# helgeanl/GP-MPC

Measured on NVIDIA H100. Metric: GP predictions/sec (N train x horizon test, fp64), higher is better.
Workload: dtype f64

## Files before the change

gp-mpc_b200/csrc/gpmpc.cu:

```cuda
#include "../../include/gpmpc.h"

#include <dlfcn.h>
#include <math.h>
#include <stdarg.h>
#include <stdlib.h>
#include <string.h>

#include <algorithm>
#include <type_traits>
#include <vector>

#include <nvtx3/nvToolsExt.h>

#include "common.cuh"
#include "gemm_dmma.cuh"
#include "predict_streamk.cuh"
#include "kernels.cuh"

#define GPMPC_VERSION 100
#define HB 64
#define NX_MAX 32
#define PSK_MAX_CTAS 2048
#define MAX_DEPTH 12
#define LOOKAHEAD_MIN_ROWS 1024

typedef struct { char internal[128]; } nccl_uid_t;
typedef void* nccl_comm_t;
struct NcclApi {
    void* lib = nullptr;
    int (*GetUniqueId)(nccl_uid_t*) = nullptr;
    int (*CommInitRank)(nccl_comm_t*, int, nccl_uid_t, int) = nullptr;
    int (*AllGather)(const void*, void*, size_t, int, nccl_comm_t, cudaStream_t) = nullptr;
    int (*CommDestroy)(nccl_comm_t) = nullptr;
    const char* (*GetErrorString)(int) = nullptr;
};
static NcclApi g_nccl;
static char g_create_err[512] = "";

static bool nccl_load(char* err, size_t errn)
{
    if (g_nccl.lib) return true;
    const char* names[] = {"libnccl.so.2", "libnccl.so"};
    for (const char* n : names) {
        g_nccl.lib = dlopen(n, RTLD_NOW | RTLD_GLOBAL);
        if (g_nccl.lib) break;
    }
    if (!g_nccl.lib) { snprintf(err, errn, "dlopen(libnccl.so.2) failed: %s", dlerror()); return false; }
    g_nccl.GetUniqueId = (int (*)(nccl_uid_t*))dlsym(g_nccl.lib, "ncclGetUniqueId");
    g_nccl.CommInitRank = (int (*)(nccl_comm_t*, int, nccl_uid_t, int))dlsym(g_nccl.lib, "ncclCommInitRank");
    g_nccl.AllGather = (int (*)(const void*, void*, size_t, int, nccl_comm_t, cudaStream_t))dlsym(g_nccl.lib, "ncclAllGather");
    g_nccl.CommDestroy = (int (*)(nccl_comm_t))dlsym(g_nccl.lib, "ncclCommDestroy");
    g_nccl.GetErrorString = (const char* (*)(int))dlsym(g_nccl.lib, "ncclGetErrorString");
    if (!g_nccl.GetUniqueId || !g_nccl.CommInitRank || !g_nccl.AllGather || !g_nccl.CommDestroy) {
        snprintf(err, errn, "libnccl is missing required symbols");
        g_nccl.lib = nullptr;
        return false;
    }
    return true;
}

template <typename T>
struct DevBuf {
    T* p = nullptr;
    size_t cap = 0;
    DevBuf() = default;
    DevBuf(const DevBuf&) = delete;
    DevBuf& operator=(const DevBuf&) = delete;
    ~DevBuf() { cudaFree(p); }
    operator T*() const { return p; }
    int ensure(gpmpc_handle_t h, long long count, const char* name);
};

struct gpmpc_handle_s {
    int N = 0, Nx = 0, Ny = 0, a0 = 0, nloc = 0, Npad = 0, device = 0;
    int nloc_max = 0;
    cudaStream_t st = nullptr;
    cudaEvent_t ev0 = nullptr, ev1 = nullptr;
    cudaStream_t sideSt[MAX_DEPTH] = {nullptr}; cudaEvent_t evA[MAX_DEPTH] = {nullptr}, evB[MAX_DEPTH] = {nullptr}, evT[MAX_DEPTH] = {nullptr}, evS[MAX_DEPTH] = {nullptr};
    long long w2off[MAX_DEPTH + 1] = {0};
    DevBuf<double> dXT, dMu, dY, dHyp, dJit, dHypTmp;
    DevBuf<double> dL, dLi, dW1, dW2;
    DevBuf<double> dAlpha, dTmp, dRes;
    DevBuf<int> dInfo;
    DevBuf<double> dKST, dPart, dPMJ, dSQ, dV, dR, dR2;
    DevBuf<unsigned int> dCnt;
    int psk_ctas = 0, opt_predict_ctas = 0;
    DevBuf<double> dCovV, dCovOut;
    DevBuf<double> dGrD;
    DevBuf<int> dGrI;
    DevBuf<double> dRm;
    DevBuf<double> dUall, dBeta, dPDV, dPH, dGradOut; bool u_valid = false;
    DevBuf<double> dDR, dVD, dPG, dPB2, dPM3, dHessOut;
    DevBuf<double> dG;
    double *dZ = nullptr, *dSigma = nullptr, *dMean = nullptr, *dVar = nullptr, *dJ = nullptr, *dCov = nullptr;
    DevBuf<double> dRoll;
    DevBuf<double> dIn, dOut;
    int Hcap = 0;
    double* hPinned = nullptr; double* dPinnedAlias = nullptr; size_t hPinnedBytes = 0;
    DevBuf<double> dU, dKinv, dGradPart, dGrad;
    bool has_data = false, has_hyper = false, factorized = false;
    DevBuf<double> dEmTr, dEMP, dEmE, dEmF, dEmW, dEmIJ;
    DevBuf<double> dEmMeanPart, dEmPart, dEmLQ, dEmVec, dEmE2, dEmF2;
    DevBuf<double> dEmKinv, dEmGPart, dEmGRec, dEmBB; bool em_kinv_valid = false;
    std::vector<double> hyper;
    std::vector<double> logdet, yalpha;
    std::vector<int> jitter_used;
    int sms = 132;
    int opt_refine = 0, opt_small_tiles = 528;
    nccl_comm_t comm = nullptr; int rank = 0, world = 1;
    DevBuf<double> dPeerBlock; long long peerGsz = 0; int peerHcap = 0; bool peer_ready = false;
    double* peerBase[GPMPC_MAXW] = {nullptr}; bool peerOpened[GPMPC_MAXW] = {false};
    int* dPeerStatus = nullptr; int* hPeerStatus = nullptr;
    unsigned long long peer_step = 0; int opt_peer = 1; double opt_peer_timeout_s = 60.0; int clock_khz = 1980000;
    char err[512] = "";
};

static void set_error(gpmpc_handle_t h, const char* fmt, ...)
{
    va_list ap; va_start(ap, fmt);
    vsnprintf(h ? h->err : g_create_err, 512, fmt, ap);
    va_end(ap);
}

template <typename T>
int DevBuf<T>::ensure(gpmpc_handle_t h, long long count, const char* name)
{
    if ((size_t)count <= cap) return GPMPC_OK;
    if (p) {
        CUDA_TRY(cudaStreamSynchronize(h->st));
        cudaFree(p);
        p = nullptr; cap = 0;
    }
    const size_t bytes = (size_t)count * sizeof(T);
    cudaError_t e = cudaMalloc((void**)&p, bytes);
    if (e != cudaSuccess) {
        p = nullptr;
        set_error(h, "cudaMalloc(%s, %zu bytes) failed: %s", name, bytes, cudaGetErrorString(e));
        return GPMPC_ERR_CUDA;
    }
    e = cudaMemsetAsync(p, 0, bytes, h->st);
    if (e != cudaSuccess) { cudaFree(p); p = nullptr; }
    CUDA_TRY(e);
    cap = (size_t)count;
    return GPMPC_OK;
}

#define ENSURE(buf, count)                                          \
    do {                                                            \
        const int _rc = (buf).ensure(h, (long long)(count), #buf);  \
        if (_rc) return _rc;                                        \
    } while (0)

struct NvtxRange {
    explicit NvtxRange(const char* name) { nvtxRangePushA(name); }
    ~NvtxRange() { nvtxRangePop(); }
};

static inline long long slab(gpmpc_handle_t h) { return (long long)h->Npad * h->Npad; }
static inline long long w2slab(gpmpc_handle_t h) { return h->w2off[MAX_DEPTH]; }

template <typename F>
static cudaError_t nxp_dispatch(int Nx, F&& f)
{
    if (Nx <= 8) return f(std::integral_constant<int, 8>());
    if (Nx <= 16) return f(std::integral_constant<int, 16>());
    return f(std::integral_constant<int, 32>());
}

static cudaError_t gemm128(gpmpc_handle_t h, cudaStream_t st, bool bt, const GemmParams& p, int batch)
{
    const long long tiles = (long long)batch * (p.lower ? (long long)p.mt * (p.mt + 1) : 2LL * p.mt * p.nt);
    GemmParams q = p;
    if (tiles < h->opt_small_tiles) {
        q.mt = p.mt * 2; q.nt = p.nt * 4;
        return bt ? gemm_launch<64, 32, 2, 2, true, 3, 4>(q, batch, st)
                  : gemm_launch<64, 32, 2, 2, false, 3, 4>(q, batch, st);
    }
    q.nt = p.nt * 2;
    if (bt && tiles >= 4LL * h->sms) return gemm_tmap_launch<128, 64, 2, 2, 4, 2>(q, batch, st);
    return bt ? gemm_launch<128, 64, 2, 2, true, 3, 2>(q, batch, st)
              : gemm_launch<128, 64, 2, 2, false, 3, 2>(q, batch, st);
}

static int potrf_inv_rec(gpmpc_handle_t h, double* A, double* Li, long long sA, long long sLi,
                         int* dInfo, int off, int n, int batch, int depth = 0, cudaEvent_t pend = nullptr)
{
    const int ld = h->Npad;
    if (n <= LEAF_N) {
        if (pend) CUDA_TRY(cudaStreamWaitEvent(h->st, pend, 0));
        CUDA_TRY(smem_opt_in<leaf_potrf_trtri_kernel>(LEAF_SMEM_DOUBLES * 8));
        leaf_potrf_trtri_kernel<<<batch, 256, LEAF_SMEM_DOUBLES * 8, h->st>>>(A + (long long)off * ld + off, ld, sA,
                                                                           Li + (long long)off * ld + off, ld, sLi, dInfo, off);
        CUDA_TRY(cudaGetLastError());
        return GPMPC_OK;
    }
    const int nb = n / GPMPC_TILE;
    const int n1 = (nb / 2) * GPMPC_TILE, n2 = n - n1;
    int rc = potrf_inv_rec(h, A, Li, sA, sLi, dInfo, off, n1, batch, depth + 1, nullptr);
    if (rc) return rc;
    if (pend) CUDA_TRY(cudaStreamWaitEvent(h->st, pend, 0));
    double* A21 = A + (long long)(off + n1) * ld + off;
    double* A22 = A + (long long)(off + n1) * ld + off + n1;
    double* Li11 = Li + (long long)off * ld + off;
    double* Li21 = Li + (long long)(off + n1) * ld + off;
    double* Li22 = Li + (long long)(off + n1) * ld + off + n1;
    double* W1 = h->dW1 + h->w2off[depth];
    double* W2 = h->dW2 + h->w2off[depth];
    const long long sW = w2slab(h), sW2 = w2slab(h);
    const bool ovl = depth < MAX_DEPTH;
    cudaStream_t side = ovl ? h->sideSt[depth] : h->st;
    const int h2 = ((n2 / GPMPC_TILE) / 2) * GPMPC_TILE;
    const bool split = ovl && h2 >= GPMPC_TILE && n >= LOOKAHEAD_MIN_ROWS;
    GemmParams p;
    auto panel = [&](cudaStream_t st, int r0, int rows) -> cudaError_t {
        GemmParams q;
        memset(&q, 0, sizeof(q));
        q.A = A21 + (long long)r0 * ld; q.lda = ld; q.sA = sA;
        q.B = Li11; q.ldb = ld; q.sB = sLi;
        q.C = W1 + (long long)r0 * n1; q.ldc = n1; q.sC = sW;
        q.mt = rows / 128; q.nt = n1 / 128; q.K = n1; q.alpha = 1.0; q.beta = 0.0; q.kflags = GEMM_KJ_LE;
        cudaError_t e = gemm128(h, st, true, q, batch);
        if (e != cudaSuccess) return e;
        dim3 g(std::max(1, std::min(64, n1 / 2 / 128)), std::min(rows, 4096), batch);
        copy2d_kernel<<<g, 128, 0, st>>>(W1 + (long long)r0 * n1, n1, sW, A21 + (long long)r0 * ld, ld, sA, rows, n1);
        return cudaGetLastError();
    };
    auto update = [&](cudaStream_t st, int r0, int rows, int c0, int cols, int lower) -> cudaError_t {
        GemmParams q;
        memset(&q, 0, sizeof(q));
        q.A = W1 + (long long)r0 * n1; q.lda = n1; q.sA = sW;
        q.B = W1 + (long long)c0 * n1; q.ldb = n1; q.sB = sW;
        q.C = A22 + (long long)r0 * ld + c0; q.ldc = ld; q.sC = sA; q.Cin = q.C; q.ldcin = ld; q.sCin = sA;
        q.mt = rows / 128; q.nt = cols / 128; q.K = n1; q.alpha = -1.0; q.beta = 1.0; q.lower = lower;
        return gemm128(h, st, true, q, batch);
    };
    if (ovl) {
        CUDA_TRY(cudaEventRecord(h->evA[depth], h->st));
        CUDA_TRY(cudaStreamWaitEvent(side, h->evA[depth], 0));
    }
    if (split) {
        CUDA_TRY(panel(h->st, 0, h2));
        CUDA_TRY(cudaEventRecord(h->evT[depth], h->st));
        CUDA_TRY(update(h->st, 0, h2, 0, h2, 1));
        CUDA_TRY(panel(side, h2, n2 - h2));
        CUDA_TRY(cudaStreamWaitEvent(side, h->evT[depth], 0));
        CUDA_TRY(update(side, h2, n2 - h2, 0, h2, 0));
        CUDA_TRY(update(side, h2, n2 - h2, h2, n2 - h2, 1));
        CUDA_TRY(cudaEventRecord(h->evS[depth], side));
    } else {
        CUDA_TRY(panel(h->st, 0, n2));
        CUDA_TRY(update(h->st, 0, n2, 0, n2, 1));
        if (ovl) {
            CUDA_TRY(cudaEventRecord(h->evT[depth], h->st));
            CUDA_TRY(cudaStreamWaitEvent(side, h->evT[depth], 0));
        }
    }
    memset(&p, 0, sizeof(p));
    p.A = A21; p.lda = ld; p.sA = sA;
    p.B = Li11; p.ldb = ld; p.sB = sLi;
    p.C = W2; p.ldc = n1; p.sC = sW2;
    p.mt = n2 / 128; p.nt = n1 / 128; p.K = n1; p.alpha = 1.0; p.beta = 0.0; p.kflags = GEMM_KJ_GE;
    if (ovl) {
        CUDA_TRY(gemm128(h, side, false, p, batch));
        CUDA_TRY(cudaEventRecord(h->evB[depth], side));
    }
    rc = potrf_inv_rec(h, A, Li, sA, sLi, dInfo, off + n1, n2, batch, depth + 1, split ? h->evS[depth] : nullptr);
    if (rc) return rc;
    if (ovl) CUDA_TRY(cudaStreamWaitEvent(h->st, h->evB[depth], 0));
    else CUDA_TRY(gemm128(h, h->st, false, p, batch));
    memset(&p, 0, sizeof(p));
    p.A = Li22; p.lda = ld; p.sA = sLi;
    p.B = W2; p.ldb = n1; p.sB = sW2;
    p.C = Li21; p.ldc = ld; p.sC = sLi;
    p.mt = n2 / 128; p.nt = n1 / 128; p.K = n2; p.alpha = -1.0; p.beta = 0.0; p.kflags = GEMM_KI_LE;
    CUDA_TRY(gemm128(h, h->st, false, p, batch));
    return GPMPC_OK;
}

static int launch_kbuild(gpmpc_handle_t h, const double* dHyp, const double* dJit, double* K, int batch, int full)
{
    const int KD = (h->Nx + 3) & ~3, S = ((KD >> 2) & 1) ? KD : KD + 4;
    const int smem = (2 * KB2_TILE * S + 2 * KB2_TILE + 256) * 8;
    const int smem_max = (2 * KB2_TILE * 36 + 2 * KB2_TILE + 256) * 8;
    CUDA_TRY(smem_opt_in<kbuild_dmma_kernel<true>>(smem_max));
    CUDA_TRY(smem_opt_in<kbuild_dmma_kernel<false>>(smem_max));
    const int T = h->Npad / KB2_TILE;
    dim3 grid(T * (T + 1) / 2, 1, batch);
    if (full)
        kbuild_dmma_kernel<true><<<grid, 256, smem, h->st>>>(h->dXT, h->Npad, h->N, h->Nx, h->dMu, dHyp, h->Nx + 2, dJit, K, h->Npad, slab(h));
    else
        kbuild_dmma_kernel<false><<<grid, 256, smem, h->st>>>(h->dXT, h->Npad, h->N, h->Nx, h->dMu, dHyp, h->Nx + 2, dJit, K, h->Npad, slab(h));
    CUDA_TRY(cudaGetLastError());
    return GPMPC_OK;
}

static int launch_alpha(gpmpc_handle_t h, int a, int batch)
{
    const int n = h->Npad;
    const double* Li = h->dLi + (long long)a * slab(h);
    dim3 g1((n + 7) / 8, 1, batch);
    trmv_lower_kernel<<<g1, 256, 0, h->st>>>(Li, n, slab(h), h->dY + (long long)a * n, n,
                                              h->dTmp + (long long)a * n, n, n);
    CUDA_TRY(cudaGetLastError());
    const int nch = (n + TRT_ROWS - 1) / TRT_ROWS;
    double* P = h->dW1 + (long long)a * w2slab(h);
    dim3 g2(n / 32, nch, batch);
    trmv_lower_T_part_kernel<<<g2, 256, 0, h->st>>>(Li, n, slab(h), h->dTmp + (long long)a * n, n, P, w2slab(h), n);
    CUDA_TRY(cudaGetLastError());
    alpha_logdet_kernel<<<batch, 1024, 0, h->st>>>(P, w2slab(h), nch, h->dL + (long long)a * slab(h), n, slab(h),
                                                   h->dY + (long long)a * n, n, h->dAlpha + (long long)a * n, n, n, h->dRes + 2 * a);
    CUDA_TRY(cudaGetLastError());
    return GPMPC_OK;
}

static int factor_one(gpmpc_handle_t h, int a, const double* dHyp, double jitter, int* used)
{
    double* L = h->dL + (long long)a * slab(h);
    double* Li = h->dLi + (long long)a * slab(h);
    *used = 0;
    for (int attempt = 0; attempt < 2; ++attempt) {
        const double jit = attempt ? jitter : 0.0;
        CUDA_TRY(cudaMemcpyAsync(h->dJit + a, &jit, sizeof(double), cudaMemcpyHostToDevice, h->st));
        CUDA_TRY(cudaMemsetAsync(h->dInfo + a, 0, sizeof(int), h->st));
        {
            int rck = launch_kbuild(h, dHyp, h->dJit + a, L, 1, 0);
            if (rck) return rck;
        }
        int rc = potrf_inv_rec(h, L, Li, slab(h), slab(h), h->dInfo + a, 0, h->Npad, 1);
        if (rc) return rc;
        int info = 0;
        CUDA_TRY(cudaMemcpyAsync(&info, h->dInfo + a, sizeof(int), cudaMemcpyDeviceToHost, h->st));
        CUDA_TRY(cudaStreamSynchronize(h->st));
        if (info == 0) { *used = attempt; return GPMPC_OK; }
        *used = 1 + info;
    }
    return GPMPC_ERR_NOTPD;
}

extern "C" int gpmpc_version(void) { return GPMPC_VERSION; }

extern "C" const char* gpmpc_last_error(gpmpc_handle_t h) { return h ? h->err : g_create_err; }

extern "C" int gpmpc_destroy(gpmpc_handle_t h);

static int create_fill(gpmpc_handle_t h, int N, int N_cap, int Nx, int Ny, int out_begin, int out_count, int device)
{
    h->N = N; h->Nx = Nx; h->Ny = Ny; h->a0 = out_begin; h->nloc = out_count; h->device = device;
    h->nloc_max = out_count; h->world = 1; h->rank = 0;
    h->Npad = (std::max(N, N_cap) + GPMPC_TILE - 1) / GPMPC_TILE * GPMPC_TILE;
    CUDA_TRY(cudaSetDevice(device));
    CUDA_TRY(cudaDeviceGetAttribute(&h->sms, cudaDevAttrMultiProcessorCount, device));
    h->opt_small_tiles = 4 * h->sms;
    h->psk_ctas = PSK_CTAS_PER_SM * h->sms;
    cudaDeviceGetAttribute(&h->clock_khz, cudaDevAttrClockRate, device);
    {
        int lo = 0, hi = 0;
        cudaDeviceGetStreamPriorityRange(&lo, &hi);
        CUDA_TRY(cudaStreamCreateWithPriority(&h->st, cudaStreamNonBlocking, hi));
    }
    CUDA_TRY(cudaEventCreate(&h->ev0));
    CUDA_TRY(cudaEventCreate(&h->ev1));
    const long long np = h->Npad;
    ENSURE(h->dXT, (long long)Nx * np);
    ENSURE(h->dMu, NX_MAX);
    ENSURE(h->dY, (long long)out_count * np);
    ENSURE(h->dHyp, (long long)out_count * (Nx + 2));
    ENSURE(h->dHypTmp, Nx + 2);
    ENSURE(h->dJit, out_count);
    ENSURE(h->dL, out_count * slab(h));
    ENSURE(h->dLi, out_count * slab(h));
    {
        const int nb = h->Npad / 128;
        long long off = 0;
        for (int d = 0; d < MAX_DEPTH; ++d) {
            h->w2off[d] = off;
            const long long nd = (long long)((nb + (1 << d) - 1) >> d) * 128;
            off += nd * nd / 4 + 128;
        }
        h->w2off[MAX_DEPTH] = off;
        int lo = 0, hi = 0;
        cudaDeviceGetStreamPriorityRange(&lo, &hi);
        for (int d = 0; d < MAX_DEPTH; ++d) {
            CUDA_TRY(cudaStreamCreateWithPriority(&h->sideSt[d], cudaStreamNonBlocking, lo));
            CUDA_TRY(cudaEventCreateWithFlags(&h->evA[d], cudaEventDisableTiming));
            CUDA_TRY(cudaEventCreateWithFlags(&h->evB[d], cudaEventDisableTiming));
            CUDA_TRY(cudaEventCreateWithFlags(&h->evT[d], cudaEventDisableTiming));
            CUDA_TRY(cudaEventCreateWithFlags(&h->evS[d], cudaEventDisableTiming));
        }
    }
    ENSURE(h->dW1, out_count * w2slab(h));
    ENSURE(h->dW2, out_count * w2slab(h));
    ENSURE(h->dAlpha, (long long)out_count * np);
    ENSURE(h->dTmp, (long long)out_count * np);
    ENSURE(h->dRes, 2 * out_count);
    ENSURE(h->dInfo, out_count);
    ENSURE(h->dGrad, Nx + 2);
    h->hyper.assign((size_t)out_count * (Nx + 2), 0.0);
    h->logdet.assign(out_count, 0.0); h->yalpha.assign(out_count, 0.0); h->jitter_used.assign(out_count, 0);
    CUDA_TRY(cudaStreamSynchronize(h->st));
    return GPMPC_OK;
}


extern "C" int gpmpc_create(int N, int Nx, int Ny, int out_begin, int out_count, int device, gpmpc_handle_t* out)
{
    return gpmpc_create_reserve(N, N, Nx, Ny, out_begin, out_count, device, out);
}

extern "C" int gpmpc_create_reserve(int N, int N_cap, int Nx, int Ny, int out_begin, int out_count, int device,
                                    gpmpc_handle_t* out)
{
    gpmpc_handle_t h = nullptr;
    if (!out) return GPMPC_ERR_ARG;
    *out = nullptr;
    if (N < 1 || Nx < 1 || Nx > NX_MAX || Ny < 1 || out_begin < 0 || out_count < 1 || out_begin + out_count > Ny) {
        set_error(nullptr, "gpmpc_create: bad sizes N=%d (capacity %d) Nx=%d (max %d) Ny=%d outputs [%d,%d)", N, N_cap, Nx,
                  NX_MAX, Ny, out_begin, out_begin + out_count);
        return GPMPC_ERR_ARG;
    }
    int ndev = 0;
    cudaError_t e = cudaGetDeviceCount(&ndev);
    if (e != cudaSuccess || ndev < 1 || device < 0 || device >= ndev) {
        set_error(nullptr, "gpmpc_create: no usable CUDA device %d (count %d, %s) -- this engine has no CPU path",
                  device, ndev, cudaGetErrorString(e));
        return GPMPC_ERR_CUDA;
    }
    cudaDeviceProp prop;
    if (cudaGetDeviceProperties(&prop, device) != cudaSuccess || prop.major != 9 || prop.minor != 0) {
        set_error(nullptr, "gpmpc_create: device %d is sm_%d%d; this library is built for sm_90a (H100) only", device,
                  prop.major, prop.minor);
        return GPMPC_ERR_CUDA;
    }
    h = new gpmpc_handle_s();
    const int rc = create_fill(h, N, N_cap, Nx, Ny, out_begin, out_count, device);
    if (rc != GPMPC_OK) {
        snprintf(g_create_err, sizeof(g_create_err), "gpmpc_create: %s", h->err);
        gpmpc_destroy(h);
        return rc;
    }
    *out = h;
    return GPMPC_OK;
}

extern "C" int gpmpc_destroy(gpmpc_handle_t h)
{
    if (!h) return GPMPC_OK;
    cudaSetDevice(h->device);
    if (h->st) cudaStreamSynchronize(h->st);
    if (h->comm && g_nccl.CommDestroy) g_nccl.CommDestroy(h->comm);
    for (int r = 0; r < GPMPC_MAXW; ++r) if (h->peerOpened[r]) cudaIpcCloseMemHandle(h->peerBase[r]);
    if (h->hPeerStatus) cudaFreeHost(h->hPeerStatus);
    if (h->hPinned) cudaFreeHost(h->hPinned);
    for (int d = 0; d < MAX_DEPTH; ++d) {
        if (h->sideSt[d]) { cudaStreamSynchronize(h->sideSt[d]); cudaStreamDestroy(h->sideSt[d]); }
        if (h->evA[d]) cudaEventDestroy(h->evA[d]);
        if (h->evB[d]) cudaEventDestroy(h->evB[d]);
        if (h->evT[d]) cudaEventDestroy(h->evT[d]);
        if (h->evS[d]) cudaEventDestroy(h->evS[d]);
    }
    if (h->ev0) cudaEventDestroy(h->ev0);
    if (h->ev1) cudaEventDestroy(h->ev1);
    if (h->st) cudaStreamDestroy(h->st);
    delete h;
    return GPMPC_OK;
}

static int ensure_pinned(gpmpc_handle_t h, size_t bytes)
{
    if (h->hPinnedBytes >= bytes) return GPMPC_OK;
    if (h->hPinned) cudaFreeHost(h->hPinned);
    h->hPinned = nullptr; h->hPinnedBytes = 0;
    CUDA_TRY(cudaHostAlloc((void**)&h->hPinned, bytes, cudaHostAllocMapped));
    CUDA_TRY(cudaHostGetDevicePointer((void**)&h->dPinnedAlias, h->hPinned, 0));
    h->hPinnedBytes = bytes;
    return GPMPC_OK;
}

static void factor_caches_stale(gpmpc_handle_t h) { h->u_valid = false; h->em_kinv_valid = false; }
static void factor_stale(gpmpc_handle_t h) { h->factorized = false; factor_caches_stale(h); }

extern "C" int gpmpc_set_data(gpmpc_handle_t h, const double* X, const double* Y)
{
    if (!h || !X || !Y) return GPMPC_ERR_ARG;
    CUDA_TRY(cudaSetDevice(h->device));
    const int N = h->N, Nx = h->Nx, np = h->Npad;
    std::vector<double> xt((size_t)Nx * np, 0.0), yl((size_t)h->nloc * np, 0.0);
    for (int i = 0; i < N; ++i)
        for (int d = 0; d < Nx; ++d) xt[(size_t)d * np + i] = X[(size_t)i * Nx + d];
    for (int a = 0; a < h->nloc; ++a)
        for (int i = 0; i < N; ++i) yl[(size_t)a * np + i] = Y[(size_t)i * h->Ny + h->a0 + a];
    double mu[NX_MAX] = {0.0};
    for (int d = 0; d < Nx; ++d) {
        double sacc = 0.0;
        for (int i = 0; i < N; ++i) sacc += X[(size_t)i * Nx + d];
        mu[d] = sacc / N;
    }
    CUDA_TRY(cudaMemcpyAsync(h->dMu, mu, NX_MAX * 8, cudaMemcpyHostToDevice, h->st));
    CUDA_TRY(cudaMemcpyAsync(h->dXT, xt.data(), xt.size() * 8, cudaMemcpyHostToDevice, h->st));
    CUDA_TRY(cudaMemcpyAsync(h->dY, yl.data(), yl.size() * 8, cudaMemcpyHostToDevice, h->st));
    CUDA_TRY(cudaStreamSynchronize(h->st));
    h->has_data = true; factor_stale(h);
    return GPMPC_OK;
}

static int local_index(gpmpc_handle_t h, int a);

// ... 122 lines not shown
    GemmParams p;
    memset(&p, 0, sizeof(p));
    p.A = h->dU; p.lda = np; p.B = h->dU; p.ldb = np; p.C = h->dKinv; p.ldc = np;
    p.mt = np / 128; p.nt = np / 128; p.K = np; p.alpha = 1.0; p.beta = 0.0;
    p.kflags = GEMM_KI_GE | GEMM_KJ_GE; p.lower = 1;
    CUDA_TRY(gemm128(h, h->st, true, p, 1));
    return GPMPC_OK;
}

template <int NXP>
static cudaError_t launch_grad(gpmpc_handle_t h, int al, const double* dHyp)
{
    const int T = h->Npad / KB_TILE;
    const int smem = 2 * h->Nx * KB_TILE * 8;
    nlml_grad_kernel<NXP><<<T * (T + 1) / 2, 256, smem, h->st>>>(h->dXT, h->Npad, h->N, h->Nx, dHyp, h->dKinv, h->Npad,
                                                                 h->dAlpha + (long long)al * h->Npad, h->dGradPart);
    return cudaGetLastError();
}

extern "C" int gpmpc_nlml(gpmpc_handle_t h, int a, const double* theta, double* nll, double* grad)
{
    if (!h || !theta || !nll) return GPMPC_ERR_ARG;
    if (!h->has_data) { set_error(h, "gpmpc_nlml: set_data first"); return GPMPC_ERR_STATE; }
    CUDA_TRY(cudaSetDevice(h->device));
    const int al = local_index(h, a);
    if (al < 0) return GPMPC_ERR_ARG;
    const int m = h->Nx + 2;
    for (int d = 0; d < h->Nx; ++d) if (theta[d] == 0.0) { set_error(h, "gpmpc_nlml: zero length scale"); return GPMPC_ERR_ARG; }
    factor_stale(h);
    NvtxRange nvtx_r("gpmpc.nlml");
    CUDA_TRY(cudaMemcpyAsync(h->dHypTmp, theta, m * 8, cudaMemcpyHostToDevice, h->st));
    int used = 0;
    int rc = factor_one(h, al, h->dHypTmp, 1e-8, &used);
    if (rc) { if (rc == GPMPC_ERR_NOTPD) set_error(h, "gpmpc_nlml: K not positive definite even with jitter"); return rc; }
    rc = launch_alpha(h, al, 1);
    if (rc) return rc;
    double res[2];
    CUDA_TRY(cudaMemcpyAsync(res, h->dRes + 2 * al, 16, cudaMemcpyDeviceToHost, h->st));
    if (grad) {
        rc = compute_kinv(h, al);
        if (rc) return rc;
        CUDA_TRY(nxp_dispatch(h->Nx, [&](auto nxp) { return launch_grad<decltype(nxp)::value>(h, al, h->dHypTmp); }));
        const int T = h->Npad / KB_TILE;
        nlml_grad_final_kernel<<<m, 256, 0, h->st>>>(h->dGradPart, T * (T + 1) / 2, h->Nx, h->dHypTmp, h->dGrad);
        CUDA_TRY(cudaGetLastError());
        CUDA_TRY(cudaMemcpyAsync(grad, h->dGrad, m * 8, cudaMemcpyDeviceToHost, h->st));
    }
    CUDA_TRY(cudaStreamSynchronize(h->st));
    *nll = 0.5 * res[1] + 0.5 * res[0];
    return GPMPC_OK;
}

extern "C" int gpmpc_get(gpmpc_handle_t h, int what, int a, double* dst)
{
    if (!h || !dst) return GPMPC_ERR_ARG;
    CUDA_TRY(cudaSetDevice(h->device));
    const int al = local_index(h, a);
    if (al < 0) return GPMPC_ERR_ARG;
    if (what == GPMPC_GET_K) return gpmpc_build_K(h, a, dst);
    if (what == GPMPC_GET_ALPHA_NLML) {
        CUDA_TRY(cudaMemcpyAsync(dst, h->dAlpha + (long long)al * h->Npad, h->N * 8, cudaMemcpyDeviceToHost, h->st));
        CUDA_TRY(cudaStreamSynchronize(h->st));
        return GPMPC_OK;
    }
    if (!h->factorized) { set_error(h, "gpmpc_get: call gpmpc_factorize first"); return GPMPC_ERR_STATE; }
    switch (what) {
    case GPMPC_GET_CHOL: return extract_to_host(h, h->dL + (long long)al * slab(h), dst, 1);
    case GPMPC_GET_LINV: return extract_to_host(h, h->dLi + (long long)al * slab(h), dst, 1);
    case GPMPC_GET_ALPHA:
        CUDA_TRY(cudaMemcpyAsync(dst, h->dAlpha + (long long)al * h->Npad, h->N * 8, cudaMemcpyDeviceToHost, h->st));
        CUDA_TRY(cudaStreamSynchronize(h->st));
        return GPMPC_OK;
    case GPMPC_GET_LOGDET: dst[0] = h->logdet[al]; return GPMPC_OK;
    case GPMPC_GET_INVK: {
        int rc = compute_kinv(h, al);
        if (rc) return rc;
        return extract_to_host(h, h->dKinv, dst, 2);
    }
    default: set_error(h, "gpmpc_get: unknown selector %d", what); return GPMPC_ERR_ARG;
    }
}

extern "C" int gpmpc_set_option(gpmpc_handle_t h, const char* name, double value)
{
    if (!h || !name) return GPMPC_ERR_ARG;
    if (!strcmp(name, "refine")) { h->opt_refine = value != 0.0; return GPMPC_OK; }
    if (!strcmp(name, "predict_ctas")) {
        const int v = (int)value;
        if (v < 0 || v > PSK_MAX_CTAS) { set_error(h, "predict_ctas must be in [0, %d]", PSK_MAX_CTAS); return GPMPC_ERR_ARG; }
        h->opt_predict_ctas = v; return GPMPC_OK;
    }
    if (!strcmp(name, "peer_timeout_s")) { h->opt_peer_timeout_s = value > 0.0 ? value : 60.0; return GPMPC_OK; }
    if (!strcmp(name, "small_tiles")) { h->opt_small_tiles = (int)value; return GPMPC_OK; }
    if (!strcmp(name, "peer")) { h->opt_peer = value != 0.0; return GPMPC_OK; }
    set_error(h, "unknown option %s", name);
    return GPMPC_ERR_ARG;
}

static inline int ks_chunk(gpmpc_handle_t h)
{
    if (h->Npad < 8192) return 128;
    return (h->nloc >= 2 && h->Nx <= 12) ? 1024 : 512;
}

static inline int ks_blocks(gpmpc_handle_t h) { return (h->Npad + ks_chunk(h) - 1) / ks_chunk(h); }

static inline int round8(int n) { return (n + 7) / 8 * 8; }

static int ensure_rows(gpmpc_handle_t h)
{
    ENSURE(h->dV, (long long)h->nloc * HB * h->Npad);
    ENSURE(h->dR, (long long)h->nloc * HB * h->Npad);
    return GPMPC_OK;
}

static int ensure_predict_bufs(gpmpc_handle_t h, int H)
{
    const long long np = h->Npad, nt = np / 128;
    ENSURE(h->dKST, (long long)h->nloc * HB * np);
    ENSURE(h->dPMJ, (long long)h->nloc * HB * ks_blocks(h) * (h->Nx + 1));
    ENSURE(h->dSQ, (long long)h->nloc * HB * nt);
    ENSURE(h->dCnt, (long long)h->nloc * nt + h->nloc + 1);
    ENSURE(h->dPart, (long long)std::max(h->psk_ctas, h->opt_predict_ctas) * 2 * HB * PSK_BN);
    if (h->opt_refine) {
        int rc = ensure_rows(h);
        if (rc) return rc;
        ENSURE(h->dR2, (long long)h->nloc * HB * np);
    }
    if (H > h->Hcap) {
        h->Hcap = 0;
        h->dZ = h->dSigma = h->dMean = h->dVar = h->dJ = h->dCov = nullptr;
        const long long cap = std::max(H, HB);
        const int nyp = h->nloc_max * h->world;
        const long long Nx = h->Nx, Ny = h->Ny;
        ENSURE(h->dG, (long long)nyp * cap * (Nx + 2));
        ENSURE(h->dIn, cap * Nx + cap * Nx * Nx);
        ENSURE(h->dOut, cap * (2 * Ny + Ny * Nx + Ny * Ny));
        h->dZ = h->dIn; h->dSigma = h->dIn + cap * Nx;
        h->dMean = h->dOut; h->dVar = h->dOut + cap * Ny; h->dJ = h->dOut + 2 * cap * Ny;
        h->dCov = h->dOut + 2 * cap * Ny + cap * Ny * Nx;
        h->Hcap = (int)cap;
    }
    return GPMPC_OK;
}

template <int BM>
static cudaError_t psk_launch_bm(const PredictParams& p, const double* A, long long sA, const double* B, long long sB,
                                 int np, int grid, cudaStream_t st)
{
    constexpr int BYTES = psk_pipe_doubles(BM) * 8 + 2 * PSK_STAGES * 8 + 1024;
    const cudaError_t e = smem_opt_in<predict_streamk_kernel<BM>>(BYTES);
    if (e != cudaSuccess) return e;
    CUtensorMap tmA, tmB;
    if (!tmap_make(&tmA, A, np, BM, np, sA, p.nloc, BM)) return cudaErrorInvalidValue;
    if (!tmap_make(&tmB, B, np, np, np, sB, p.nloc, PSK_BN)) return cudaErrorInvalidValue;
    cudaLaunchConfig_t cfg;
    memset(&cfg, 0, sizeof(cfg));
    cfg.gridDim = dim3(grid); cfg.blockDim = dim3(PSK_THREADS); cfg.dynamicSmemBytes = BYTES; cfg.stream = st;
    cudaLaunchAttribute attr[1];
    attr[0].id = cudaLaunchAttributeProgrammaticStreamSerialization;
    attr[0].val.programmaticStreamSerializationAllowed = 1;
    cfg.attrs = attr; cfg.numAttrs = 1;
    return cudaLaunchKernelEx(&cfg, predict_streamk_kernel<BM>, p, tmA, tmB);
}

static int psk_grid(gpmpc_handle_t h, long long G)
{
    int ctas = h->opt_predict_ctas > 0 ? h->opt_predict_ctas : h->psk_ctas;
    ctas = std::min(ctas, PSK_MAX_CTAS);
    const long long by_work = std::max(1LL, G / 4);
    return (int)std::min<long long>(ctas, h->opt_predict_ctas > 0 ? G : by_work);
}

static cudaError_t psk_launch(gpmpc_handle_t h, const PredictParams& p, const double* A, const double* B)
{
    const long long sA = (long long)HB * h->Npad, sB = slab(h);
    const int np = h->Npad, grid = psk_grid(h, p.G);
    switch (round8(p.Hc)) {
    case 8: return psk_launch_bm<8>(p, A, sA, B, sB, np, grid, h->st);
    case 16: return psk_launch_bm<16>(p, A, sA, B, sB, np, grid, h->st);
    case 24: return psk_launch_bm<24>(p, A, sA, B, sB, np, grid, h->st);
    case 32: return psk_launch_bm<32>(p, A, sA, B, sB, np, grid, h->st);
    case 40: return psk_launch_bm<40>(p, A, sA, B, sB, np, grid, h->st);
    case 48: return psk_launch_bm<48>(p, A, sA, B, sB, np, grid, h->st);
    case 56: return psk_launch_bm<56>(p, A, sA, B, sB, np, grid, h->st);
    default: return psk_launch_bm<64>(p, A, sA, B, sB, np, grid, h->st);
    }
}

static void psk_base(gpmpc_handle_t h, PredictParams& p, int Hc, int upper = 0)
{
    memset(&p, 0, sizeof(p));
    const long long nt = h->Npad / 128;
    p.nloc = h->nloc; p.nt = (int)nt; p.Hc = Hc; p.upper = upper;
    p.ntb = (int)((h->Npad + PSK_BN - 1) / PSK_BN); p.nk = h->Npad / GEMM_BK;
    p.T = psk_steps_per_output(p.ntb, p.nk, upper); p.G = p.T * h->nloc;
    p.part = h->dPart;
    p.tile_cnt = h->dCnt; p.out_cnt = h->dCnt + (long long)h->nloc * nt; p.done_cnt = p.out_cnt + h->nloc;
    p.SQ = h->dSQ;
    p.hyp = h->dHyp; p.hyp_ld = h->Nx + 2; p.Nx = h->Nx;
}

static void psk_finalize(gpmpc_handle_t h, PredictParams& p, int H, int h0)
{
    p.finalize = 1; p.PMJ = h->dPMJ; p.nblk_mj = ks_blocks(h);
    p.Gloc = h->dG; p.slot0 = h->a0; p.Htot = H; p.h0 = h0;
}

static AssembleArgs assemble_args(gpmpc_handle_t h, int H, int method, const double* Sigma, int spp,
                                  double* mean, double* var, double* J, double* cov)
{
    AssembleArgs as;
    memset(&as, 0, sizeof(as));
    as.G = h->dG; as.Ny = h->Ny; as.Nx = h->Nx; as.H = H; as.method_ta = (method == GPMPC_METHOD_TA);
    as.Sigma = Sigma; as.sigma_per_point = spp;
    as.mean = mean; as.var = var; as.J = J; as.cov = cov;
    as.world = 1;
    as.stage_g = (assemble_rows_doubles(H, h->Ny, h->Nx) <= psk_pipe_doubles(round8(std::min(H, HB)))) ? 1 : 0;
    return as;
}

template <int NXP, int CH>
static cudaError_t launch_ks(gpmpc_handle_t h, const double* dZc, int Hc)
{
    const int smem = (NXP + 1) * CH * 8, nblk = ks_blocks(h);
    const cudaError_t e = smem_opt_in<ks_tile_kernel<NXP, CH>>(smem);
    if (e != cudaSuccess) return e;
    dim3 g(nblk, round8(Hc) / 8, h->nloc);
    ks_tile_kernel<NXP, CH><<<g, 256, smem, h->st>>>(h->dXT, h->Npad, h->N, h->Nx, h->dHyp, h->Nx + 2, h->dAlpha, h->Npad,
                                                     dZc, Hc, h->dKST, h->Npad, (long long)HB * h->Npad, h->dPMJ, nblk);
    return cudaGetLastError();
}

template <int CH>
static cudaError_t launch_ks_nx(gpmpc_handle_t h, const double* dZc, int Hc)
{
    const int Nx = h->Nx;
    if (Nx <= 4) return launch_ks<4, CH>(h, dZc, Hc);
    if (Nx <= 6) return launch_ks<6, CH>(h, dZc, Hc);
    if (Nx <= 8) return launch_ks<8, CH>(h, dZc, Hc);
    if (Nx <= 10) return launch_ks<10, CH>(h, dZc, Hc);
    if (Nx <= 12) return launch_ks<12, CH>(h, dZc, Hc);
    if (CH <= 512) {
        if (Nx <= 16) return launch_ks<16, (CH <= 512 ? CH : 512)>(h, dZc, Hc);
        if (Nx <= 24) return launch_ks<24, (CH <= 512 ? CH : 512)>(h, dZc, Hc);
        return launch_ks<32, (CH <= 512 ? CH : 512)>(h, dZc, Hc);
    }
    return cudaErrorInvalidValue;
}

static cudaError_t launch_ks(gpmpc_handle_t h, const double* dZc, int Hc)
{
    switch (ks_chunk(h)) {
    case 1024: return launch_ks_nx<1024>(h, dZc, Hc);
    case 512: return launch_ks_nx<512>(h, dZc, Hc);
    default: return launch_ks_nx<128>(h, dZc, Hc);
    }
}

static int tri_product(gpmpc_handle_t h, const double* Amat, const double* T, int Hc, double* Vout)
{
    PredictParams p;
    psk_base(h, p, Hc);
    p.Vout = Vout; p.sV = (long long)HB * h->Npad; p.ldv = h->Npad;
    CUDA_TRY(psk_launch(h, p, Amat, T));
    return GPMPC_OK;
}

__global__ void axpby_rows_kernel(const double* __restrict__ x, const double* __restrict__ y, double a, double b,
                                  double* __restrict__ out, long long rowlen, long long srow, int rows)
{
    const long long i = (long long)blockIdx.x * blockDim.x + threadIdx.x;
    const int r = blockIdx.y, bz = blockIdx.z;
    if (i >= rowlen || r >= rows) return;
    const long long o = (long long)bz * srow + (long long)r * rowlen + i;
    out[o] = a * x[o] + b * y[o];
}

static int predict_core(gpmpc_handle_t h, int method, int H, const double* dZ, const double* dSigma, int spp,
                        double* d_mean, double* d_var, double* d_cov, double* d_jac)
{
    const int np = h->Npad, Nx = h->Nx;
    NvtxRange nvtx_r("gpmpc.predict");
    const int use_peers = (h->world > 1 && h->peer_ready && h->opt_peer && H <= h->peerHcap) ? 1 : 0;
    const int nccl_gather = (h->world > 1 && !use_peers) ? 1 : 0;
    const long long timeout_clocks = (long long)(h->opt_peer_timeout_s * 1e3 * (double)h->clock_khz);
    PeerArgs pa;
    memset(&pa, 0, sizeof(pa));
    if (use_peers) {
        h->peer_step += 1;
        for (int r = 0; r < h->world; ++r) pa.base[r] = h->peerBase[r];
        pa.world = h->world; pa.rank = h->rank;
        pa.goff = 2 * GPMPC_MAXW + (long long)(h->peer_step & 1) * h->peerGsz;
        pa.flag_idx = (int)(h->peer_step & 1) * GPMPC_MAXW + h->rank;
        pa.step = h->peer_step;
        pa.timeout_clocks = timeout_clocks;
    }
    AssembleArgs as = assemble_args(h, H, method, dSigma, spp, d_mean, d_var, d_jac, d_cov);
    if (use_peers) as.G = h->dPeerBlock + pa.goff;
    as.flags = use_peers ? reinterpret_cast<const unsigned long long*>(h->dPeerBlock.p) + (h->peer_step & 1) * GPMPC_MAXW : nullptr;
    as.world = h->world; as.step = h->peer_step; as.status = h->dPeerStatus; as.timeout_clocks = timeout_clocks;
    const bool fused_assemble = (H <= HB) && !nccl_gather && ((long long)H * h->Ny * Nx * 8 <= 64 * 1024);
    for (int h0 = 0; h0 < H; h0 += HB) {
        const int Hc = std::min(HB, H - h0);
        const bool last_chunk = (h0 + HB >= H);
        const double* dZc = dZ + (long long)h0 * Nx;
        CUDA_TRY(launch_ks(h, dZc, Hc));
        PredictParams p;
        psk_base(h, p, Hc);
        psk_finalize(h, p, H, h0);
        p.pa = pa; p.use_peers = use_peers; p.publish = last_chunk ? 1 : 0;
        p.as = as; p.do_assemble = (fused_assemble && !h->opt_refine) ? 1 : 0;
        if (!h->opt_refine) {
            CUDA_TRY(psk_launch(h, p, h->dKST, h->dLi));
        } else {
            int rc = tri_product(h, h->dKST, h->dLi, Hc, h->dV);
            if (rc) return rc;
            rc = tri_product(h, h->dV, h->dL, Hc, h->dR);
            if (rc) return rc;
            const int bm = round8(Hc);
            dim3 g((np + 255) / 256, bm, h->nloc);
            axpby_rows_kernel<<<g, 256, 0, h->st>>>(h->dKST, h->dR, 1.0, -1.0, h->dR, np, (long long)HB * np, bm);
            CUDA_TRY(cudaGetLastError());
            rc = tri_product(h, h->dR, h->dLi, Hc, h->dR2);
            if (rc) return rc;
            axpby_rows_kernel<<<g, 256, 0, h->st>>>(h->dV, h->dR2, 1.0, 1.0, h->dV, np, (long long)HB * np, bm);
            CUDA_TRY(cudaGetLastError());
            sq_rows_kernel<<<dim3(np / 128, Hc, h->nloc), 128, 0, h->st>>>(h->dV, np, (long long)HB * np, h->dSQ, np / 128);
            CUDA_TRY(cudaGetLastError());
            finalize_kernel<<<h->nloc, PSK_THREADS, 0, h->st>>>(p);
            CUDA_TRY(cudaGetLastError());
        }
    }
    if (nccl_gather) {
        const size_t cnt = (size_t)h->nloc_max * H * (Nx + 2);
        int r = g_nccl.AllGather(h->dG + (size_t)h->rank * cnt, h->dG, cnt, 8 , h->comm, h->st);
        if (r) { set_error(h, "ncclAllGather failed: %s", g_nccl.GetErrorString ? g_nccl.GetErrorString(r) : "?"); return GPMPC_ERR_NCCL; }
    }
    if (!fused_assemble || h->opt_refine) {
        const int smem = (2 * h->Ny * Nx + h->Ny) * 8;
// ... 940 lines not shown
    if (n >= N) { set_error(h, "gpmpc_remove: removing %d of %d points leaves none", n, N); return GPMPC_ERR_ARG; }
    std::vector<int> order(idx, idx + n);
    std::sort(order.begin(), order.end(), [](int u, int v) { return u > v; });
    if (order[0] >= N || order[n - 1] < 0) { set_error(h, "gpmpc_remove: index out of range [0, %d)", N); return GPMPC_ERR_ARG; }
    for (int k = 1; k < n; ++k)
        if (order[k] == order[k - 1]) { set_error(h, "gpmpc_remove: index %d given twice", order[k]); return GPMPC_ERR_ARG; }
    CUDA_TRY(cudaSetDevice(h->device));
    int rc = ensure_nlml_scratch(h);
    if (rc) return rc;
    ENSURE(h->dRm, (long long)nl * 3 * np);
    NvtxRange nvtx_r("gpmpc.remove");
    const dim3 gcol((np + 255) / 256);
    for (int k = 0; k < n; ++k) {
        const int i = order[k], Nk = N - k, m = Nk - i - 1;
        if (m > 0) {
            remove_coef_kernel<<<nl, 1024, 0, h->st>>>(h->dL, h->dLi, np, slab(h), i, m, h->dRm);
            CUDA_TRY(cudaGetLastError());
        }
        for (int a = 0; a < nl; ++a) {
            double* L = h->dL + (long long)a * slab(h);
            double* Li = h->dLi + (long long)a * slab(h);
            const double* coef = h->dRm + (long long)a * 3 * np;
            if (m > 0) {
                const int nb = (m + RM_RB - 1) / RM_RB;
                remove_l_rows_kernel<<<m, 256, 0, h->st>>>(L, h->dU, np, coef, i, m);
                CUDA_TRY(cudaGetLastError());
                remove_li_part_kernel<<<dim3(gcol.x, nb), 256, 0, h->st>>>(Li, np, coef, i, m, h->dW1);
                CUDA_TRY(cudaGetLastError());
                remove_li_scan_kernel<<<gcol, 256, 0, h->st>>>(h->dW1, np, nb);
                CUDA_TRY(cudaGetLastError());
                remove_li_apply_kernel<<<dim3(gcol.x, nb), 256, 0, h->st>>>(Li, h->dKinv, np, coef, i, m, h->dW1);
                CUDA_TRY(cudaGetLastError());
            }
            remove_commit_kernel<<<m + 1, 256, 0, h->st>>>(L, Li, h->dU, h->dKinv, np, i, Nk);
            CUDA_TRY(cudaGetLastError());
        }
        remove_shift_kernel<<<Nx + nl, 256, 0, h->st>>>(h->dXT, Nx, h->dY, np, i, Nk);
        CUDA_TRY(cudaGetLastError());
    }
    h->N = N - n;
    factor_caches_stale(h);
    rc = launch_alpha(h, 0, nl);
    if (rc) return rc;
    std::vector<double> res(2 * nl);
    CUDA_TRY(cudaMemcpyAsync(res.data(), h->dRes, 2 * nl * 8, cudaMemcpyDeviceToHost, h->st));
    CUDA_TRY(cudaStreamSynchronize(h->st));
    for (int a = 0; a < nl; ++a) { h->logdet[a] = res[2 * a]; h->yalpha[a] = res[2 * a + 1]; }
    return GPMPC_OK;
}

extern "C" int gpmpc_comm_unique_id(void* id128)
{
    if (!id128) return GPMPC_ERR_ARG;
    if (!nccl_load(g_create_err, sizeof(g_create_err))) return GPMPC_ERR_NCCL;
    nccl_uid_t id;
    int r = g_nccl.GetUniqueId(&id);
    if (r) { snprintf(g_create_err, sizeof(g_create_err), "ncclGetUniqueId failed (%d)", r); return GPMPC_ERR_NCCL; }
    memcpy(id128, &id, 128);
    return GPMPC_OK;
}

extern "C" int gpmpc_comm_init(gpmpc_handle_t h, const void* id128, int rank, int world)
{
    if (!h || !id128 || world < 1 || rank < 0 || rank >= world) return GPMPC_ERR_ARG;
    CUDA_TRY(cudaSetDevice(h->device));
    const int nlm = (h->Ny + world - 1) / world;
    if (h->a0 != std::min(h->Ny, rank * nlm) || h->nloc > nlm) {
        set_error(h, "gpmpc_comm_init: rank %d of %d must own outputs starting at %d (at most %d); handle owns [%d,%d)",
                  rank, world, rank * nlm, nlm, h->a0, h->a0 + h->nloc);
        return GPMPC_ERR_ARG;
    }
    if (world > 1) {
        if (!nccl_load(h->err, sizeof(h->err))) return GPMPC_ERR_NCCL;
        nccl_uid_t id;
        memcpy(&id, id128, 128);
        int r = g_nccl.CommInitRank(&h->comm, world, id, rank);
        if (r) { set_error(h, "ncclCommInitRank failed: %s", g_nccl.GetErrorString ? g_nccl.GetErrorString(r) : "?"); return GPMPC_ERR_NCCL; }
    }
    h->rank = rank; h->world = world; h->nloc_max = nlm;
    h->Hcap = 0;
    return GPMPC_OK;
}

extern "C" int gpmpc_peer_export(gpmpc_handle_t h, int Hcap, void* handle64)
{
    if (!h || !handle64 || Hcap < 1) return GPMPC_ERR_ARG;
    CUDA_TRY(cudaSetDevice(h->device));
    if (h->world > GPMPC_MAXW) { set_error(h, "peer exchange supports at most %d ranks", GPMPC_MAXW); return GPMPC_ERR_ARG; }
    if (h->dPeerBlock) { set_error(h, "gpmpc_peer_export: already exported"); return GPMPC_ERR_STATE; }
    const int nyp = h->nloc_max * h->world;
    h->peerGsz = (long long)nyp * Hcap * (h->Nx + 2);
    h->peerHcap = Hcap;
    ENSURE(h->dPeerBlock, 2 * GPMPC_MAXW + 2 * h->peerGsz);
    if (!h->dPeerStatus) {
        CUDA_TRY(cudaHostAlloc((void**)&h->hPeerStatus, sizeof(int), cudaHostAllocMapped));
        *h->hPeerStatus = 0;
        CUDA_TRY(cudaHostGetDevicePointer((void**)&h->dPeerStatus, h->hPeerStatus, 0));
    }
    CUDA_TRY(cudaStreamSynchronize(h->st));
    cudaIpcMemHandle_t mh;
    CUDA_TRY(cudaIpcGetMemHandle(&mh, h->dPeerBlock));
    static_assert(sizeof(cudaIpcMemHandle_t) == 64, "IPC handle size");
    memcpy(handle64, &mh, 64);
    return GPMPC_OK;
}

extern "C" int gpmpc_peer_attach(gpmpc_handle_t h, const void* handles)
{
    if (!h || !handles) return GPMPC_ERR_ARG;
    if (!h->dPeerBlock) { set_error(h, "gpmpc_peer_attach: call gpmpc_peer_export first"); return GPMPC_ERR_STATE; }
    CUDA_TRY(cudaSetDevice(h->device));
    for (int r = 0; r < h->world; ++r) {
        if (r == h->rank) { h->peerBase[r] = h->dPeerBlock; continue; }
        cudaIpcMemHandle_t mh;
        memcpy(&mh, (const char*)handles + 64 * r, 64);
        void* ptr = nullptr;
        CUDA_TRY(cudaIpcOpenMemHandle(&ptr, mh, cudaIpcMemLazyEnablePeerAccess));
        h->peerBase[r] = (double*)ptr; h->peerOpened[r] = true;
    }
    h->peer_ready = true; h->peer_step = 0;
    return GPMPC_OK;
}

extern "C" int gpmpc_get_size(gpmpc_handle_t h, int* N, int* Nx, int* Ny)
{
    if (!h) return GPMPC_ERR_ARG;
    if (N) *N = h->N;
    if (Nx) *Nx = h->Nx;
    if (Ny) *Ny = h->Ny;
    return GPMPC_OK;
}

extern "C" void* gpmpc_stream(gpmpc_handle_t h) { return h ? (void*)h->st : nullptr; }

extern "C" int gpmpc_synchronize(gpmpc_handle_t h)
{
    if (!h) return GPMPC_ERR_ARG;
    CUDA_TRY(cudaSetDevice(h->device));
    CUDA_TRY(cudaStreamSynchronize(h->st));
    return peer_status_check(h);
}

template <typename Setup>
static int profile_product(gpmpc_handle_t h, const char* fn, int H, const double* out, bool all_outputs, int n_tail,
                           Setup&& setup, std::vector<unsigned long long>& t, int* grid)
{
    if (!h || !out || H < 1 || H > HB) return GPMPC_ERR_ARG;
    int rc = predict_guard(h, fn, GPMPC_METHOD_TA, H);
    if (rc) return rc;
    rc = predict_prepare(h, fn, HB, all_outputs);
    if (rc) return rc;
    PredictParams p;
    psk_base(h, p, H);
    *grid = psk_grid(h, p.G);
    DevBuf<unsigned long long> dbg;
    ENSURE(dbg, (long long)*grid * 2 + n_tail);
    p.dbg = dbg;
    setup(p, dbg + 2 * *grid);
    for (int rep = 0; rep < 2; ++rep) {
        const cudaError_t e = psk_launch(h, p, h->dKST, h->dLi);
        if (e != cudaSuccess) { set_error(h, "%s: %s", fn, cudaGetErrorString(e)); return GPMPC_ERR_CUDA; }
    }
    t.resize((size_t)*grid * 2 + n_tail);
    cudaMemcpyAsync(t.data(), dbg, t.size() * 8, cudaMemcpyDeviceToHost, h->st);
    cudaStreamSynchronize(h->st);
    return GPMPC_OK;
}

extern "C" int gpmpc_profile_balance(gpmpc_handle_t h, int H, double* out4)
{
    std::vector<unsigned long long> t; int grid = 0;
    const int rc = profile_product(h, __func__, H, out4, false, 0, [](PredictParams&, unsigned long long*) {}, t, &grid);
    if (rc) return rc;
    unsigned long long lo = ~0ull, hi = 0; double mn = 1e300, mx = 0.0, sum = 0.0;
    for (int c = 0; c < grid; ++c) {
        const double d = (double)(t[2 * c + 1] - t[2 * c]) * 1e-3;
        mn = std::min(mn, d); mx = std::max(mx, d); sum += d;
        lo = std::min(lo, t[2 * c]); hi = std::max(hi, t[2 * c + 1]);
    }
    out4[0] = mn; out4[1] = mx; out4[2] = sum / grid; out4[3] = (double)(hi - lo) * 1e-3;
    return GPMPC_OK;
}

extern "C" int gpmpc_profile_tail(gpmpc_handle_t h, int H, double* out8)
{
    std::vector<unsigned long long> t; int grid = 0;
    auto setup = [&](PredictParams& p, unsigned long long* tail) {
        psk_finalize(h, p, H, 0);
        p.as = assemble_args(h, H, GPMPC_METHOD_TA, h->dSigma, 0, h->dMean, h->dVar, h->dJ, h->dCov);
        p.as.dbg = tail;
        p.do_assemble = 1;
    };
    const int rc = profile_product(h, __func__, H, out8, true, 8, setup, t, &grid);
    if (rc) return rc;
    unsigned long long lo = ~0ull, hi = 0, hi2 = 0; int cmax = 0;
    for (int c = 0; c < grid; ++c) {
        lo = std::min(lo, t[2 * c]);
        if (t[2 * c + 1] > hi) { hi2 = hi; hi = t[2 * c + 1]; cmax = c; } else hi2 = std::max(hi2, t[2 * c + 1]);
    }
    for (int k = 0; k < 6; ++k) out8[k] = ((double)t[2 * grid + k] - (double)hi2) * 1e-3;
    out8[6] = (double)(hi - lo) * 1e-3;
    out8[7] = (double)(t[2 * cmax + 1] - t[2 * cmax]) * 1e-3;
    return GPMPC_OK;
}

extern "C" int gpmpc_profile_leaf(gpmpc_handle_t h, double* out15)
{
    if (!h || !out15) return GPMPC_ERR_ARG;
    if (!h->has_data || !h->has_hyper) { set_error(h, "gpmpc_profile_leaf: set_data and set_hyper first"); return GPMPC_ERR_STATE; }
    CUDA_TRY(cudaSetDevice(h->device));
    DevBuf<long long> d;
    ENSURE(d, 16);
    CUDA_TRY(cudaMemcpyToSymbol(d_leaf_prof, &d.p, sizeof(d.p)));
    int rc = GPMPC_OK;
    for (int rep = 0; rep < 2 && rc == GPMPC_OK; ++rep) {
        rc = launch_kbuild(h, h->dHyp, h->dJit, h->dL, 1, 0);
        if (rc == GPMPC_OK) rc = potrf_inv_rec(h, h->dL, h->dLi, slab(h), slab(h), h->dInfo, 0, 128, 1);
    }
    cudaStreamSynchronize(h->st);
    long long hst[16];
    cudaMemcpy(hst, d, sizeof(hst), cudaMemcpyDeviceToHost);
    long long* nul = nullptr;
    cudaMemcpyToSymbol(d_leaf_prof, &nul, sizeof(nul));
    for (int k = 0; k < 15; ++k) out15[k] = (double)(hst[k] - hst[0]);
    factor_stale(h);
    return rc;
}

extern "C" int gpmpc_profile(gpmpc_handle_t h, int what, int n, int reps, double* ms_out)
{
    if (!h || !ms_out || reps < 1) return GPMPC_ERR_ARG;
    if (!h->has_data || !h->has_hyper) { set_error(h, "gpmpc_profile: set_data and set_hyper first"); return GPMPC_ERR_STATE; }
    CUDA_TRY(cudaSetDevice(h->device));
    const int np = h->Npad, Hc = (n > 0 && n <= HB) ? n : 56;
    float ms = 0.f;
    int rc = GPMPC_OK;
    auto run = [&]() -> int {
        switch (what) {
        case GPMPC_PROF_KBUILD_FULL: return launch_kbuild(h, h->dHyp, h->dJit, h->dL, 1, 1);
        case GPMPC_PROF_KBUILD_LOWER: return launch_kbuild(h, h->dHyp, h->dJit, h->dL, 1, 0);
        case GPMPC_PROF_SYRK: {
            const int nn = (n > 0 && n <= np) ? n / 128 * 128 : np;
            const int n1 = (nn / 128 / 2) * 128, n2 = nn - n1;
            if (n1 < 128) { set_error(h, "gpmpc_profile: SYRK needs N >= 256"); return GPMPC_ERR_ARG; }
            GemmParams p;
            memset(&p, 0, sizeof(p));
            p.A = h->dW1; p.lda = n1; p.B = h->dW1; p.ldb = n1;
            p.C = h->dLi; p.ldc = np; p.Cin = h->dLi; p.ldcin = np;
            p.mt = n2 / 128; p.nt = n2 / 128; p.K = n1; p.alpha = -1e-30; p.beta = 1.0; p.lower = 1;
            cudaError_t e = gemm128(h, h->st, true, p, 1);
            if (e != cudaSuccess) { set_error(h, "profile syrk: %s", cudaGetErrorString(e)); return GPMPC_ERR_CUDA; }
            return GPMPC_OK;
        }
        case GPMPC_PROF_FACTORIZE: {
            int r = launch_kbuild(h, h->dHyp, h->dJit, h->dL, 1, 0);
            if (r) return r;
            return potrf_inv_rec(h, h->dL, h->dLi, slab(h), slab(h), h->dInfo, 0, np, 1);
        }
        case GPMPC_PROF_TRIGEMM: return tri_product(h, h->dKST, h->dLi, Hc, nullptr);
        case GPMPC_PROF_KS: {
            cudaError_t e = launch_ks(h, h->dZ, Hc);
            if (e != cudaSuccess) { set_error(h, "profile ks: %s", cudaGetErrorString(e)); return GPMPC_ERR_CUDA; }
            return GPMPC_OK;
        }
        case GPMPC_PROF_PREDICT_TAIL: {
            PredictParams p;
            psk_base(h, p, Hc);
            psk_finalize(h, p, Hc, 0);
            p.as = assemble_args(h, Hc, GPMPC_METHOD_TA, h->dSigma, 0, h->dMean, h->dVar, h->dJ, h->dCov);
            p.do_assemble = (h->world == 1 && h->nloc == h->Ny) ? 1 : 0;
            cudaError_t e = psk_launch(h, p, h->dKST, h->dLi);
            if (e != cudaSuccess) { set_error(h, "profile predict tail: %s", cudaGetErrorString(e)); return GPMPC_ERR_CUDA; }
            return GPMPC_OK;
        }
        default: set_error(h, "gpmpc_profile: unknown selector %d", what); return GPMPC_ERR_ARG;
        }
    };
    const bool product = what == GPMPC_PROF_TRIGEMM || what == GPMPC_PROF_KS || what == GPMPC_PROF_PREDICT_TAIL;
    if (product) { rc = ensure_predict_bufs(h, HB); if (rc) return rc; }
    CUDA_TRY(cudaMemsetAsync(h->dJit, 0, h->nloc * sizeof(double), h->st));
    rc = run();
    if (rc) return rc;
    CUDA_TRY(cudaStreamSynchronize(h->st));
    CUDA_TRY(cudaEventRecord(h->ev0, h->st));
    for (int r = 0; r < reps; ++r) { rc = run(); if (rc) return rc; }
    CUDA_TRY(cudaEventRecord(h->ev1, h->st));
    CUDA_TRY(cudaEventSynchronize(h->ev1));
    CUDA_TRY(cudaEventElapsedTime(&ms, h->ev0, h->ev1));
    ms_out[0] = (double)ms / reps;
    if (!product) factor_stale(h);
    return GPMPC_OK;
}
```

Baseline: 14780.

## Split stream-K predict launch into L2-sized output rounds

Queries the device L2 size and splits the stream-K predict kernel across groups of outputs, so each launch's A operand slabs fit in about three quarters of L2 and get reused from cache rather than DRAM. Intermediate rounds turn off publish, assemble and debug, and per-round pointers are offset into SQ, PMJ, hyp, Vout and the slot indices. The A tensor map now uses the real horizon Hc as its row extent instead of the padded BM, which avoids loading padding rows. The cost is extra launches and smaller grids per round, which may underfill the GPU, and correctness depends on counter and offset handling across rounds.

```diff
diff --git a/gp-mpc_b200/csrc/gpmpc.cu b/gp-mpc_b200/csrc/gpmpc.cu
--- a/gp-mpc_b200/csrc/gpmpc.cu
+++ b/gp-mpc_b200/csrc/gpmpc.cu
@@ -85,6 +85,7 @@
     DevBuf<double> dKST, dPart, dPMJ, dSQ, dV, dR, dR2;
     DevBuf<unsigned int> dCnt;
     int psk_ctas = 0, opt_predict_ctas = 0;
+    int l2_bytes = 0;
     DevBuf<double> dCovV, dCovOut;
     DevBuf<double> dGrD;
     DevBuf<int> dGrI;
@@ -352,6 +353,7 @@
     CUDA_TRY(cudaDeviceGetAttribute(&h->sms, cudaDevAttrMultiProcessorCount, device));
     h->opt_small_tiles = 4 * h->sms;
     h->psk_ctas = PSK_CTAS_PER_SM * h->sms;
+    CUDA_TRY(cudaDeviceGetAttribute(&h->l2_bytes, cudaDevAttrL2CacheSize, device));
     cudaDeviceGetAttribute(&h->clock_khz, cudaDevAttrClockRate, device);
     {
         int lo = 0, hi = 0;
@@ -780,7 +782,7 @@
     const cudaError_t e = smem_opt_in<predict_streamk_kernel<BM>>(BYTES);
     if (e != cudaSuccess) return e;
     CUtensorMap tmA, tmB;
-    if (!tmap_make(&tmA, A, np, BM, np, sA, p.nloc, BM)) return cudaErrorInvalidValue;
+    if (!tmap_make(&tmA, A, np, p.Hc, np, sA, p.nloc, BM)) return cudaErrorInvalidValue;
     if (!tmap_make(&tmB, B, np, np, np, sB, p.nloc, PSK_BN)) return cudaErrorInvalidValue;
     cudaLaunchConfig_t cfg;
     memset(&cfg, 0, sizeof(cfg));
@@ -800,20 +802,45 @@
     return (int)std::min<long long>(ctas, h->opt_predict_ctas > 0 ? G : by_work);
 }
 
+#define PSK_L2_SHARE 0.75
+static int psk_rounds(gpmpc_handle_t h, int nloc)
+{
+    const long long fit = (long long)(PSK_L2_SHARE * h->l2_bytes) / ((long long)HB * h->Npad * 8);
+    const int R = (int)std::max(1LL, std::min<long long>(nloc, fit));
+    return (nloc + R - 1) / R;
+}
+static inline int psk_round_begin(int nloc, int r, int n) { return (int)((long long)nloc * r / n); }
+
 static cudaError_t psk_launch(gpmpc_handle_t h, const PredictParams& p, const double* A, const double* B)
 {
     const long long sA = (long long)HB * h->Npad, sB = slab(h);
-    const int np = h->Npad, grid = psk_grid(h, p.G);
-    switch (round8(p.Hc)) {
-    case 8: return psk_launch_bm<8>(p, A, sA, B, sB, np, grid, h->st);
-    case 16: return psk_launch_bm<16>(p, A, sA, B, sB, np, grid, h->st);
-    case 24: return psk_launch_bm<24>(p, A, sA, B, sB, np, grid, h->st);
-    case 32: return psk_launch_bm<32>(p, A, sA, B, sB, np, grid, h->st);
-    case 40: return psk_launch_bm<40>(p, A, sA, B, sB, np, grid, h->st);
-    case 48: return psk_launch_bm<48>(p, A, sA, B, sB, np, grid, h->st);
-    case 56: return psk_launch_bm<56>(p, A, sA, B, sB, np, grid, h->st);
-    default: return psk_launch_bm<64>(p, A, sA, B, sB, np, grid, h->st);
-    }
+    const int np = h->Npad, n = psk_rounds(h, p.nloc);
+    for (int r = 0; r < n; ++r) {
+        const int r0 = psk_round_begin(p.nloc, r, n), r1 = psk_round_begin(p.nloc, r + 1, n);
+        PredictParams q = p;
+        q.nloc = r1 - r0; q.G = p.T * q.nloc;
+        q.SQ = p.SQ + (long long)r0 * 64 * p.nt;
+        if (p.PMJ) q.PMJ = p.PMJ + (long long)r0 * p.Hc * p.nblk_mj * (p.Nx + 1);
+        q.hyp = p.hyp + (long long)r0 * p.hyp_ld;
+        if (p.Vout) q.Vout = p.Vout + r0 * p.sV;
+        q.slot0 = p.slot0 + r0;
+        if (r + 1 < n) { q.publish = 0; q.do_assemble = 0; q.dbg = nullptr; q.as.dbg = nullptr; }
+        const double* Ar = A + r0 * sA; const double* Br = B + r0 * sB;
+        const int grid = psk_grid(h, q.G);
+        cudaError_t e;
+        switch (round8(p.Hc)) {
+        case 8: e = psk_launch_bm<8>(q, Ar, sA, Br, sB, np, grid, h->st); break;
+        case 16: e = psk_launch_bm<16>(q, Ar, sA, Br, sB, np, grid, h->st); break;
+        case 24: e = psk_launch_bm<24>(q, Ar, sA, Br, sB, np, grid, h->st); break;
+        case 32: e = psk_launch_bm<32>(q, Ar, sA, Br, sB, np, grid, h->st); break;
+        case 40: e = psk_launch_bm<40>(q, Ar, sA, Br, sB, np, grid, h->st); break;
+        case 48: e = psk_launch_bm<48>(q, Ar, sA, Br, sB, np, grid, h->st); break;
+        case 56: e = psk_launch_bm<56>(q, Ar, sA, Br, sB, np, grid, h->st); break;
+        default: e = psk_launch_bm<64>(q, Ar, sA, Br, sB, np, grid, h->st); break;
+        }
+        if (e != cudaSuccess) return e;
+    }
+    return cudaSuccess;
 }
 
 static void psk_base(gpmpc_handle_t h, PredictParams& p, int Hc, int upper = 0)
@@ -2060,7 +2087,8 @@
     if (rc) return rc;
     PredictParams p;
     psk_base(h, p, H);
-    *grid = psk_grid(h, p.G);
+    const int n = psk_rounds(h, p.nloc);
+    *grid = psk_grid(h, p.T * (p.nloc - psk_round_begin(p.nloc, n - 1, n)));
     DevBuf<unsigned long long> dbg;
     ENSURE(dbg, (long long)*grid * 2 + n_tail);
     p.dbg = dbg;
```

Result: faster. 15290, median of 6 (+3.5%).
